# google-deepmind/dm_control

Measured on AMD Instinct MI355X. Metric: env-steps/s (whole node) at batch 4096; max rel qpos error vs CPU, higher is better.
Workload: dtype f32

## Files before the change

### dm_control_amd/csrc/step_core.h

```cpp
#pragma once
#include "../../include/dmc_model_layout.h"
#include "step_layout.h"
#include "step_defs.h"
#include "step_math.h"
#include "step_lanes.h"
#include "step_dense.h"
#include "step_geom.h"

namespace dmc {
#ifdef DMC_HOST_EMU
inline int& emu_split_solves() { static int n = 0; return n; }
inline long long* emu_ls_counts() { static long long n[6] = {0, 0, 0, 0, 0, 0}; return n; }
#endif

#if defined(DMC_PROFILE) && !defined(DMC_HOST_EMU)
#define DMC_PROF(id) do { if (lane == 0) { const int t_ = (int)__builtin_readcyclecounter(); SI(prof)[id] += t_ - SI(prof)[33]; SI(prof)[33] = t_; } } while (0)
#else
#define DMC_PROF(id) ((void)0)
#endif
#ifdef DMC_TRACE_SUB
#define DMC_TSUB(region, cond, row) do { if (DMC_TRACE_SUB == (region) && (cond)) sub_stamp(row); } while (0)
#else
#define DMC_TSUB(region, cond, row) ((void)0)
#endif
enum { PROF_LOAD = 0, PROF_KIN, PROF_COM, PROF_CRB, PROF_COLL, PROF_CONSTR, PROF_COMVEL, PROF_RNE, PROF_SENS, PROF_ACT,
       PROF_ACC, PROF_SOL_INIT, PROF_SOL_GRAD, PROF_SOL_LS, PROF_SOL_UPD, PROF_EULER, PROF_TRAIL, PROF_STORE,
       PROF_NOSLIP, PROF_HESS, PROF_FACTOR, PROF_SOLVE, PROF_LS_SETUP, PROF_X1, PROF_X2, PROF_X3, PROF_X4, PROF_X5, PROF_X6,
       PROF_X7, PROF_X8, PROF_N };

enum {
  OUT_SENSOR = 1 << 0, OUT_XPOS = 1 << 1, OUT_XQUAT = 1 << 2, OUT_XMAT = 1 << 3,
  OUT_XIPOS = 1 << 4, OUT_GEOM = 1 << 5, OUT_SITE = 1 << 6, OUT_SUBTREE_COM = 1 << 7,
  OUT_QACC = 1 << 8, OUT_ACTUATOR = 1 << 9, OUT_CONTACT = 1 << 10, OUT_QFRC = 1 << 11, OUT_CVEL = 1 << 12,
  OUT_CONTACT_IDS = 1 << 13,
  OUT_ALL = 0x7fffffff
};

enum LaunchMode { MODE_STEP = 0, MODE_FORWARD = 1, MODE_FORWARD_NOACT = 2, MODE_ROLLOUT = 3, MODE_STEP1 = 4, MODE_STEP2 = 5 };

template <typename T>
struct StepIO {
  int B;
  T *qpos, *qvel, *ctrl, *qacc_warmstart, *qfrc_applied;
  T *act;
  double* time;
  T *sensordata, *xpos, *xquat, *xmat, *xipos, *geom_xpos, *geom_xmat;
  T *site_xpos, *site_xmat, *subtree_com, *qacc, *actuator_force, *qfrc_actuator;
  T *qfrc_bias, *qfrc_constraint, *contact_dist, *contact_pos, *contact_frame;
  T *contact_force;
  T *cvel;
  int *ncon, *nefc, *solver_iter, *warning, *contact_geom1, *contact_geom2;
  const int* env_mode;
  int* work;
  int* cost; const int* order;
  int* prog = nullptr; int slices = 0; int nxcd = 1;
  unsigned long long* hand = nullptr; int hand_n = 0;
  const void* task_args = nullptr;
  int* trace; int trace_slot;
  T* probe = nullptr; int probe_geom = 0, probe_cap = 0;
  const T* ctrl_seq; T *qpos_seq, *qvel_seq, *sensor_seq;
  T* stash_r; int* stash_i; const int* epoch;
  T* kstash; int* kstash_i;
  long long* prof;
  T* debug;
  int* debug_i;
  int ndebug;
};

#ifndef DMC_STATIC_FEATURES
#define DMC_STATIC_FEATURES 1
#endif
template <typename T> struct LSPoint { T alpha, cost, d0, d1; };
template <typename T> DMC_DEV constexpr bool ls_relative() { return sizeof(T) == 4; }
template <typename T> DMC_DEV constexpr bool ls_anchored() { return ls_relative<T>(); }
#ifdef DMC_HOST_EMU
template <typename T> struct LSVec { T v[4]; DMC_DEV T operator[](int i) const { return v[i]; } };
#define DMC_LSVEC(T) LSVec<T>
#else
#define DMC_LSVEC(T) T __attribute__((ext_vector_type(4)))
#endif
template <typename T, int LPE>
DMC_FN DMC_LSVEC(T) ls_eval_lds(T a, const DMC_LDS T* jar_, const DMC_LDS T* jv_, const DMC_LDS T* D_,
                                T qg0, T qg1, T qg2, int nefc, int lane) {
  LSPoint<T> pt;
  LSPoint<T>* p = &pt;
  p->alpha = a;
  T q0 = 0, q1 = 0, q2 = 0;
  for (int i = lane; i < nefc; i += LPE) {
    const T jar = jar_[i], jv = jv_[i];
    if (ls_relative<T>()) {
      const bool act_a = jar + a*jv < 0, act_0 = jar < 0;
      if (act_a | act_0) {
        const T D = D_[i], dj0 = D*jar;
        if (act_a) { if (!ls_anchored<T>()) q1 += jv*dj0; q2 += (T)0.5*D*jv*jv; }
        if (act_a != act_0) { q0 += (act_a ? (T)0.5 : (T)-0.5)*jar*dj0; if (ls_anchored<T>()) q1 += act_a ? jv*dj0 : -(jv*dj0); }
      }
    } else if (jar + a*jv < 0) {
      const T D = D_[i], dj0 = D*jar;
      q0 += (T)0.5*jar*dj0; q1 += jv*dj0; q2 += (T)0.5*D*jv*jv;
    }
  }
  q0 = group_sum<LPE>(q0) + qg0; q1 = group_sum<LPE>(q1) + qg1; q2 = group_sum<LPE>(q2) + qg2;
  p->cost = a*a*q2 + a*q1 + q0;
  p->d0 = 2*a*q2 + q1;
  p->d1 = 2*q2;
  if (p->d1 <= 0) p->d1 = (T)DMC_MINVAL;
  DMC_LSVEC(T) rv = {pt.alpha, pt.cost, pt.d0, pt.d1};
  return rv;
}

struct DynLayoutSrc {
  static constexpr int kNV = 0;
  static constexpr int kJGlobal = -1;
  static constexpr int kNKin = 0;
  static constexpr int kTreeMax = 0;
  static constexpr int kTreeUni = 0;
  const StepLayout* p;
  DMC_DEV const StepLayout& get() const { return *p; }
};

#ifndef DMC_LS_SLOPE_ULPS
#define DMC_LS_SLOPE_ULPS 16
#endif
#ifndef DMC_PRIO_ITER
#define DMC_PRIO_ITER 2
#endif
template <typename T, int LPE, typename LS> struct StageFns;

template <typename T>
struct TaskLds { const T *qpos, *qvel, *ctrl, *act, *sensordata, *xpos, *xmat, *xipos, *subtree_com, *geom_xpos, *cvel; };

template <typename T, int LPE, typename LS = DynLayoutSrc>
struct StepCore {
  LS ls;
  const StepLayout& L;
  const StepOpts<T>& o;
  const int* mi;
  const T* mr;
  const int* gc;
  T* s;
  int* si;
  int lane;
  double time_;
  bool hsplit;


  DMC_DEV StepCore(LS ls_, const StepOpts<T>& o_, const int* mi_, const T* mr_, const int* gc_, T* s_, int* si_, int lane_)
      : ls(ls_), L(ls_.get()), o(o_), mi(mi_), mr(mr_),
#ifndef DMC_HOST_EMU
        gc(ls_.get().d.coldlds ? reinterpret_cast<const int*>(mr_ + ls_.get().n_mr_lds) : gc_),
#else
        gc(gc_),
#endif
        s(s_), si(si_), lane(lane_), time_(0), hsplit(false) {}

#define MI(n) (mi + L.mi_##n)
#define MR(n) (mr + L.mr_##n)
#define MRC(n) (mrc() + L.mr_##n)
#define MRS(n) ((L.d.sitegl ? (const T*)o.g_mr : (const T*)mr) + L.mr_##n)
#define GC(n) (gc + L.mc_##n)
#define S(n) (s + L.s_##n)
#define SG(n) (sg_##n())
#define SI(n) (si + L.si_##n)
#define FOR_LANES(i, n) for (int i = lane; i < (n); i += LPE)

// ... 2556 lines not shown
    chol_factor_inplace(S(qLH), nv, hsplit);
    DMC_PROF(PROF_FACTOR);
    chol_solve(S(sv_Mgrad), S(qLH), S(sv_grad), nv, hsplit);
    DMC_PROF(PROF_SOLVE);
  }
  DMC_DEV bool h_split(int nefc) {
    if (!L.d.treemax) return false;
    const RowMap rm = row_map();
    if (rm.s0 > 0 || rm.c0 > rm.tl0) return false;
    const int ncon = rm.c0 < nefc ? SI(imisc)[IM_NCON] : 0;
    int coupled = 0;
    for (int c = lane; c < ncon; c += LPE) {
      if (SI(con_efc)[c] < 0) continue;
      const unsigned lo = con_mask_lo(c), hi = con_mask_hi(c);
      if (!(lo | hi)) continue;
      const int first = lo ? __builtin_ctz(lo) : 32 + __builtin_ctz(hi);
      const int last = hi ? 63 - __builtin_clz(hi) : 31 - __builtin_clz(lo);
      if (last >= MI(dof_tree1)[first]) coupled = 1;
    }
    return group_max<LPE>(coupled) == 0;
  }
  typedef dmc::LSPoint<T> LSPoint;
  enum { LSK_NONE = 0, LSK_EQUALITY, LSK_FRICTION, LSK_ONESIDED, LSK_CONE };
#if !defined(DMC_NO_ROW_REDUCE)
  static constexpr int kRegsRed = LPE < 16 ? LPE : 16;
#else
  static constexpr int kRegsRed = LPE;
#endif
  struct LSRows { T jar, jv, D; bool on; bool gen; int kind; T f, rf, U0, V0, UU, UV, VV, mu, b0, b1, b2, Dm, NT0, T0; bool bottom0, middle0; };
  DMC_DEV void ls_load_gen(LSRows& g, int nefc) {
    g.gen = true; g.kind = LSK_NONE;
    g.f = g.rf = g.U0 = g.V0 = g.UU = g.UV = g.VV = g.mu = g.b0 = g.b1 = g.b2 = g.Dm = g.NT0 = g.T0 = 0; g.bottom0 = g.middle0 = false;
    const bool in = lane < nefc;
    const int i = in ? lane : 0;
    const int tid = SI(efc_tid)[i], ty = EFC_TYPE(tid), id = EFC_ID(tid);
    const bool ell = in && ty == EFC_ELLIPTIC;
    const int c = ell ? id : 0;
    const int r0 = SI(con_efc)[c], info = SI(con_info)[c];
    const bool head = ell && i == r0;
    T jr[6], jvv[6], Dr[6];
#pragma unroll
    for (int j = 0; j < 6; j++) {
#ifdef DMC_HOST_EMU
      const int rj = i + j < L.d.njmax ? i + j : i;
#else
      const int rj = i + j;
#endif
      jr[j] = S(efc_jar)[rj]; jvv[j] = S(efc_jv)[rj]; Dr[j] = S(efc_D)[rj];
    }
    const T floss = MR(dof_frictionloss)[(in && ty == EFC_FRICTION) ? id : 0];
    const T* fr = MR(prm_friction) + 3*(head ? prm_of_info(info) : 0);
    const T fr0 = fr[0], fr1 = fr[1], fr2 = fr[2];
    if (!in) return;
    g.jar = jr[0]; g.jv = jvv[0]; g.D = Dr[0];
    if (ty == EFC_EQUALITY) { g.kind = LSK_EQUALITY; return; }
    if (ty == EFC_FRICTION) { g.kind = LSK_FRICTION; g.f = floss; g.rf = g.f / g.D; return; }
    if (ty != EFC_ELLIPTIC) { g.kind = LSK_ONESIDED; return; }
    if (!head) return;
    g.kind = LSK_CONE;
    const int dim = info & 0xff;
    const T D0 = g.D;
    const T mu = fr0 * t_sqrt(D0 / Dr[1]);
    T UU = 0, UV = 0, VV = 0, b0 = 0, b1 = 0, b2 = 0;
#pragma unroll
    for (int j = 0; j < 6; j++) if (j < dim) {
      const T jar = jr[j], jv = jvv[j], D = Dr[j], dj0 = D*jar;
      b0 += (T)0.5*jar*dj0; b1 += jv*dj0; b2 += (T)0.5*D*jv*jv;
      if (j) {
        const T f = j < 3 ? fr0 : (j == 3 ? fr1 : fr2);
        const T u = jar*f, v = jv*f;
        UU += u*u; UV += u*v; VV += v*v;
      }
    }
    g.U0 = g.jar*mu; g.V0 = g.jv*mu; g.UU = UU; g.UV = UV; g.VV = VV; g.mu = mu; g.b0 = b0; g.b1 = b1; g.b2 = b2;
    g.Dm = D0 / t_max((T)DMC_MINVAL, mu*mu*(1 + mu*mu));
    if (UU <= 0) g.bottom0 = g.U0 < 0;
    else {
      const T T0 = t_sqrt(UU);
      if (g.U0 >= mu*T0) {}
      else if (mu*g.U0 + T0 <= 0) g.bottom0 = true;
      else { g.middle0 = true; g.NT0 = g.U0 - mu*T0; g.T0 = T0; }
    }
  }
  DMC_DEV void ls_eval_gen(LSPoint* p, const T* qg, const LSRows& g) {
    const T a = p->alpha;
    constexpr bool rel = ls_relative<T>();
    const bool anch = anchored();
    T q0 = 0, q1 = 0, q2 = 0, cc = 0, cd0 = 0, cd1 = 0;
    if (g.kind == LSK_EQUALITY) {
      const T dj0 = g.D*g.jar;
      if (!rel) q0 += (T)0.5*g.jar*dj0;
      if (!anch) q1 += g.jv*dj0;
      q2 += (T)0.5*g.D*g.jv*g.jv;
    } else if (g.kind == LSK_FRICTION) {
      const T jar = g.jar, jv = g.jv, D = g.D, f = g.f, rf = g.rf, x = jar + a*jv;
      const int za = x <= -rf ? -1 : (x >= rf ? 1 : 0), z0 = jar <= -rf ? -1 : (jar >= rf ? 1 : 0);
      if (za < 0) { q0 += f*((T)-0.5*rf - jar); if (!anch) q1 += -f*jv; }
      else if (za > 0) { q0 += f*((T)-0.5*rf + jar); if (!anch) q1 += f*jv; }
      else { const T dj0 = D*jar; q0 += (T)0.5*jar*dj0; if (!anch) q1 += jv*dj0; q2 += (T)0.5*D*jv*jv; }
      if (rel) {
        if (z0 < 0) q0 -= f*((T)-0.5*rf - jar);
        else if (z0 > 0) q0 -= f*((T)-0.5*rf + jar);
        else q0 -= (T)0.5*jar*D*jar;
      }
      if (anch && za != z0) q1 += (za < 0 ? -f*jv : (za > 0 ? f*jv : jv*(D*jar))) - (z0 < 0 ? -f*jv : (z0 > 0 ? f*jv : jv*(D*jar)));
    } else if (g.kind == LSK_ONESIDED) {
      const T jar = g.jar, jv = g.jv;
      if (rel) {
        const bool act_a = jar + a*jv < 0, act_0 = jar < 0;
        if (act_a | act_0) {
          const T D = g.D, dj0 = D*jar;
          if (act_a) { if (!anch) q1 += jv*dj0; q2 += (T)0.5*D*jv*jv; }
          if (act_a != act_0) { q0 += (act_a ? (T)0.5 : (T)-0.5)*jar*dj0; if (anch) q1 += act_a ? jv*dj0 : -(jv*dj0); }
        }
      } else if (jar + a*jv < 0) { const T D = g.D, dj0 = D*jar; q0 += (T)0.5*jar*dj0; q1 += jv*dj0; q2 += (T)0.5*D*jv*jv; }
    } else if (g.kind == LSK_CONE) {
      const T U0 = g.U0, V0 = g.V0, UU = g.UU, UV = g.UV, VV = g.VV, mu = g.mu, Dm = g.Dm;
      const T N = U0 + a*V0, Tsqr = UU + a*(2*UV + a*VV);
      bool bottom = false, middle = false;
      T NT = 0, NT1 = 0, Tn = 0;
      if (Tsqr <= 0) bottom = N < 0;
      else {
        Tn = t_sqrt(Tsqr);
        if (N >= mu*Tn) {}
        else if (mu*N + Tn <= 0) bottom = true;
        else {
          middle = true;
          const T N1 = V0, T1 = (UV + a*VV)/Tn, T2 = VV/Tn - (UV + a*VV)*T1/(Tn*Tn);
          NT1 = N1 - mu*T1;
          NT = N - mu*Tn;
          if (!rel) cc += (T)0.5*Dm*NT*NT;
          if (!anch) cd0 += Dm*NT*NT1;
          cd1 += Dm*(NT1*NT1 - NT*mu*T2);
        }
      }
      if (!rel) { if (bottom) { q0 += g.b0; q1 += g.b1; q2 += g.b2; } }
      else {
        if (bottom) { if (!anch || !g.bottom0) q1 += g.b1; q2 += g.b2; if (!g.bottom0) q0 += g.b0; }
        else if (g.bottom0) q0 -= g.b0;
        if (anch && g.bottom0 && !bottom) q1 -= g.b1;
        if (middle | g.middle0) {
          if (!anch) cc += (T)0.5*Dm*(NT - g.NT0)*(NT + g.NT0);
          else cone_middle_anchored(a, middle, g.middle0, Dm, NT, NT1, Tn, g.NT0, g.T0, V0, UV, VV, mu, &cc, &cd0);
        }
      }
    }
    q0 = group_sum<LPE>(q0) + (rel ? (T)0 : qg[0]); q1 = group_sum<LPE>(q1) + qg[1]; q2 = group_sum<LPE>(q2) + qg[2];
    cc = group_sum<LPE>(cc); cd0 = group_sum<LPE>(cd0); cd1 = group_sum<LPE>(cd1);
    p->cost = a*a*q2 + a*q1 + q0 + cc;
    p->d0 = 2*a*q2 + q1 + cd0;
    p->d1 = 2*q2 + cd1;
    if (p->d1 <= 0) p->d1 = (T)DMC_MINVAL;
  }
  template <int RED = LPE>
  DMC_DEV void ls_eval(LSPoint* p, const T* qg, int nefc, int* evals, const LSRows& rw) {
#ifdef DMC_HOST_EMU
    emu_ls_counts()[1]++;
#endif
    if (general_rows()) { if (rw.gen) ls_eval_gen(p, qg, rw); else ls_eval_ell(p, qg, nefc); (*evals)++; return; }
    if (rw.on) {
      const T a = p->alpha, jar = rw.jar, jv = rw.jv;
      T q0 = 0, q1 = 0, q2 = 0;
      if (ls_relative<T>()) {
        const bool act_a = jar + a*jv < 0, act_0 = jar < 0;
        if (act_a | act_0) {
          const T D = rw.D, dj0 = D*jar;
          if (act_a) { if (!ls_anchored<T>()) q1 += jv*dj0; q2 += (T)0.5*D*jv*jv; }
          if (act_a != act_0) { q0 += (act_a ? (T)0.5 : (T)-0.5)*jar*dj0; if (ls_anchored<T>()) q1 += act_a ? jv*dj0 : -(jv*dj0); }
        }
      } else if (jar + a*jv < 0) {
        const T D = rw.D, dj0 = D*jar;
        q0 += (T)0.5*jar*dj0; q1 += jv*dj0; q2 += (T)0.5*D*jv*jv;
      }
      q0 = group_sum<RED>(q0) + (ls_relative<T>() ? (T)0 : qg[0]); q1 = group_sum<RED>(q1) + qg[1]; q2 = group_sum<RED>(q2) + qg[2];
      p->cost = a*a*q2 + a*q1 + q0;
      p->d0 = 2*a*q2 + q1;
      p->d1 = 2*q2;
      if (p->d1 <= 0) p->d1 = (T)DMC_MINVAL;
      (*evals)++;
      return;
    }
    const DMC_LSVEC(T) rv = ls_eval_lds<T, LPE>(p->alpha, (const DMC_LDS T*)S(efc_jar), (const DMC_LDS T*)S(efc_jv),
                                                (const DMC_LDS T*)S(efc_D), ls_relative<T>() ? (T)0 : qg[0], qg[1], qg[2], nefc, lane);
    p->alpha = rv[0]; p->cost = rv[1]; p->d0 = rv[2]; p->d1 = rv[3];
    (*evals)++;
  }
  template <int RED = LPE>
  DMC_DEV int ls_update_bracket(LSPoint* p, const LSPoint* cand, LSPoint* pnext, const T* qg, int nefc, int* evals, const LSRows& rw) {
    int flag = 0;
    for (int i = 0; i < 3; i++) {
      if (p->d0 < 0 && cand[i].d0 < 0 && p->d0 < cand[i].d0) { *p = cand[i]; flag = 1; }
      else if (p->d0 > 0 && cand[i].d0 > 0 && p->d0 > cand[i].d0) { *p = cand[i]; flag = 2; }
    }
    if (flag) { pnext->alpha = p->alpha - p->d0/p->d1; ls_eval<RED>(pnext, qg, nefc, evals, rw); }
    return flag;
  }
  struct LSPre { T a1, a2, a3, a4, jar, jv, D; };
  template <bool REGS = false>
  DMC_DEV T primal_search(int nefc, T gauss, T scale, T* lscost, const LSPre& pre = LSPre()) {
    *lscost = 0;
    constexpr int RED = REGS ? kRegsRed : LPE;
#ifdef DMC_HOST_EMU
    emu_ls_counts()[0]++;
#endif
    const int nv = L.d.nv;
    if constexpr (!REGS) {
    mul_M(S(sv_Mv), S(sv_search));
    { const RowMap rm = row_map(); for (int i = lane; i < nefc; i += LPE) S(efc_jv)[i] = row_dot(i, S(sv_search), rm); }
    DMC_WSYNC();
    }
    LSRows rw;
    rw.jar = rw.jv = rw.D = 0; rw.on = false; rw.gen = false; rw.kind = LSK_NONE;
    if (general_rows() && nefc <= LPE && LPE > 1) ls_load_gen(rw, nefc);
    if (L.d.elliptic && !rw.gen) ls_prepare_ell(nefc);
    T a1 = 0, a2 = 0, a3 = 0, a4 = 0;
    const bool anch = anchored();
    if constexpr (REGS) { a1 = pre.a1; a2 = pre.a2; a3 = pre.a3; a4 = pre.a4; } else
    FOR_LANES(i, nv) {
      const T sr = S(sv_search)[i];
      if (anch) a1 += sr*S(sv_grad)[i];
      else { a1 += sr*S(sv_Ma)[i]; a2 += S(qfrc_smooth)[i]*sr; }
      a3 += sr*S(sv_Mv)[i]; a4 += sr*sr;
    }
    a1 = group_sum<RED>(a1); if (!anch) a2 = group_sum<RED>(a2); a3 = group_sum<RED>(a3); a4 = group_sum<RED>(a4);
    T qg[3] = {gauss, a1 - a2, (T)0.5*a3};
    const T snorm = t_sqrt(a4);
    if (snorm < (T)DMC_MINVAL) return 0;
    T gtol = o.tolerance * o.ls_tolerance * snorm / scale;
    const int lsmax = o.ls_iterations;
    int evals = 0;
#ifndef DMC_HOST_EMU
    if constexpr (REGS) { rw.on = true; rw.jar = pre.jar; rw.jv = pre.jv; rw.D = pre.D; } else
    if (!general_rows() && nefc <= LPE) {
      rw.on = true;
      if (lane < nefc) { rw.jar = S(efc_jar)[lane]; rw.jv = S(efc_jv)[lane]; rw.D = S(efc_D)[lane]; }
    }
#endif
    DMC_PROF(PROF_LS_SETUP);
    LSPoint p0, p1, p2, pmid, p1next, p2next;
    p0.alpha = 0; ls_eval<RED>(&p0, qg, nefc, &evals, rw);
#ifdef DMC_HOST_EMU
    { const char* u = getenv("DMC_LS_SLOPE_ULPS");
      if (sizeof(T) == 4) gtol = t_max(gtol, (T)((u ? atof(u) : (double)DMC_LS_SLOPE_ULPS) * 1.1920929e-7) * t_abs(p0.d0)); }
#else
    if (sizeof(T) == 4) gtol = t_max(gtol, (T)(DMC_LS_SLOPE_ULPS * 1.1920929e-7) * t_abs(p0.d0));
#endif
    p1.alpha = p0.alpha - p0.d0/p0.d1; ls_eval<RED>(&p1, qg, nefc, &evals, rw);
#ifdef DMC_HOST_EMU
    if (getenv("DMC_EMU_TRACE_LS")) fprintf(stderr, "    ls: p0 cost %.6e d0 %.6e d1 %.6e | p1 alpha %.9e cost %.6e d0 %.6e d1 %.6e | gtol %.3e qg1 %.6e\n",
                                           (double)p0.cost, (double)p0.d0, (double)p0.d1, (double)p1.alpha, (double)p1.cost, (double)p1.d0, (double)p1.d1, (double)gtol, (double)qg[1]);
#endif
    if (p0.cost < p1.cost) p1 = p0;
    if (t_abs(p1.d0) < gtol) { *lscost = p1.cost; return p1.alpha; }
    const int dir = p1.d0 < 0 ? 1 : -1;
    int p2update = 0;
    p2 = p1;
    while (p1.d0*dir <= -gtol && evals < lsmax) {
      p2 = p1; p2update = 1;
      p1.alpha -= p1.d0/p1.d1; ls_eval<RED>(&p1, qg, nefc, &evals, rw);
      if (t_abs(p1.d0) < gtol) { *lscost = p1.cost; return p1.alpha; }
    }
    if (evals >= lsmax) { *lscost = p1.cost; return p1.alpha; }
    if (!p2update) { *lscost = p1.cost; return p1.alpha; }
    p2next = p1;
    p1next.alpha = p1.alpha - p1.d0/p1.d1; ls_eval<RED>(&p1next, qg, nefc, &evals, rw);
    while (evals < lsmax) {
      pmid.alpha = (T)0.5*(p1.alpha + p2.alpha); ls_eval<RED>(&pmid, qg, nefc, &evals, rw);
      LSPoint cand[3] = {p1next, p2next, pmid};
      bool found = false; T best_cost = 0, best_alpha = 0;
      for (int i = 0; i < 3; i++) if (t_abs(cand[i].d0) < gtol && (!found || cand[i].cost < best_cost)) {
        found = true; best_cost = cand[i].cost; best_alpha = cand[i].alpha;
      }
      if (found) { *lscost = best_cost; return best_alpha; }
      const int b1 = ls_update_bracket<RED>(&p1, cand, &p1next, qg, nefc, &evals, rw);
      const int b2 = ls_update_bracket<RED>(&p2, cand, &p2next, qg, nefc, &evals, rw);
      if (!b1 && !b2) { if (pmid.cost < p0.cost) { *lscost = pmid.cost; return pmid.alpha; } return 0; }
    }
    if (p1.cost <= p2.cost && p1.cost < p0.cost) { *lscost = p1.cost; return p1.alpha; }
    if (p2.cost <= p1.cost && p2.cost < p0.cost) { *lscost = p2.cost; return p2.alpha; }
    return 0;
  }
  template <int N>
  DMC_DEV static int qcqp(T* res, const T* Ain, const T* bin, const T* dd, T r) {
    constexpr bool fast = sizeof(T) == 4;
    T A[N*N], b[N], Lc[N*N], inv[N], v[N], pv[N], la = 0;
#pragma unroll
    for (int i = 0; i < N; i++) { v[i] = 0; pv[i] = 0; inv[i] = 0; b[i] = bin[i]*dd[i]; }
#pragma unroll
    for (int i = 0; i < N; i++)
#pragma unroll
      for (int j = 0; j < N; j++) { A[i*N + j] = Ain[i*N + j]*dd[i]*dd[j]; Lc[i*N + j] = 0; }
    const T val_floor = fast ? t_max((T)1e-10, (T)(16*1.1920929e-7)*r*r) : (T)1e-10;
    bool fail = false;
    for (int iter = 0; iter < 20; iter++) {
#pragma unroll
      for (int i = 0; i < N; i++)
#pragma unroll
        for (int j = 0; j <= i; j++) {
          T t = A[i*N + j] + (i == j ? la : (T)0);
#pragma unroll
          for (int k = 0; k < j; k++) t -= Lc[i*N + k]*Lc[j*N + k];
          if (i == j) {
            if (t < (T)1e-10) fail = true;
            const T tc = t_max(t, (T)1e-30);
            if (fast) { inv[i] = t_rsqrt(tc); Lc[i*N + i] = tc*inv[i]; }
            else Lc[i*N + i] = t_sqrt(tc);
          } else Lc[i*N + j] = fast ? t*inv[j] : t/Lc[j*N + j];
        }
      if (fail) break;
#pragma unroll
      for (int i = 0; i < N; i++) {
        T t = -b[i];
#pragma unroll
        for (int k = 0; k < i; k++) t -= Lc[i*N + k]*v[k];
        v[i] = fast ? t*inv[i] : t/Lc[i*N + i];
      }
#pragma unroll
      for (int i = N - 1; i >= 0; i--) {
        T t = v[i];
#pragma unroll
        for (int k = i + 1; k < N; k++) t -= Lc[k*N + i]*v[k];
        v[i] = fast ? t*inv[i] : t/Lc[i*N + i];
      }
      T val = -r*r;
#pragma unroll
      for (int i = 0; i < N; i++) val += v[i]*v[i];
      if (val < val_floor) break;
#pragma unroll
      for (int i = 0; i < N; i++) {
        T t = v[i];
#pragma unroll
        for (int k = 0; k < i; k++) t -= Lc[i*N + k]*pv[k];
        pv[i] = fast ? t*inv[i] : t/Lc[i*N + i];
      }
      T deriv = 0;
#pragma unroll
      for (int i = 0; i < N; i++) deriv += pv[i]*pv[i];
      deriv *= -2;
      const T delta = -val/deriv;
      if (delta < (fast ? t_max((T)1e-10, (T)(4*1.1920929e-7)*la) : (T)1e-10)) break;
      la += delta;
#ifdef DMC_HOST_EMU
      emu_ls_counts()[5]++;
#endif
    }
#ifdef DMC_HOST_EMU
    emu_ls_counts()[4]++;
#endif
    if (fail) {
#pragma unroll
      for (int i = 0; i < N; i++) res[i] = 0;
      return 0;
    }
#pragma unroll
    for (int i = 0; i < N; i++) res[i] = v[i]*dd[i];
    return la != 0;
  }
  template <int N>
  DMC_DEV void noslip_block_solve(const T* Ac, const T* old, const T* bres, T* fnew, int t, int id) {
    if (N == 1) {
      const T fl = MR(dof_frictionloss)[id];
      fnew[0] = old[0] - bres[0]/Ac[0];
      if (fnew[0] < -fl) fnew[0] = -fl; else if (fnew[0] > fl) fnew[0] = fl;
    } else if (t == EFC_PYRAMIDAL) {
      const T bc0 = bres[0] - Ac[0]*old[0] - Ac[1]*old[N > 1 ? 1 : 0], bc1 = bres[N > 1 ? 1 : 0] - Ac[N > 1 ? N : 0]*old[0] - Ac[N > 1 ? N + 1 : 0]*old[N > 1 ? 1 : 0];
      const T mid = (T)0.5*(old[0] + old[N > 1 ? 1 : 0]);
      const T K1 = Ac[0] + Ac[N > 1 ? N + 1 : 0] - Ac[N > 1 ? 1 : 0] - Ac[N > 1 ? N : 0], K0 = mid*(Ac[0] - Ac[N > 1 ? N + 1 : 0]) + bc0 - bc1;
      T f0, f1;
      if (K1 < (T)DMC_MINVAL) f0 = f1 = mid;
      else {
        const T y = -K0/K1;
        if (y < -mid) { f0 = 0; f1 = 2*mid; }
        else if (y > mid) { f0 = 2*mid; f1 = 0; }
        else { f0 = mid + y; f1 = mid - y; }
      }
      fnew[0] = f0; fnew[N > 1 ? 1 : 0] = f1;
    } else {
      const T* fr3 = MR(prm_friction) + 3*con_prm(id);
      const T fri5[5] = {fr3[0], fr3[0], fr3[1], fr3[2], fr3[2]};
      T fri[N], bc[N];
#pragma unroll
      for (int p = 0; p < N; p++) fri[p] = fri5[p < 5 ? p : 4];
      const T fn = S(efc_force)[SI(con_efc)[id]];
#pragma unroll
      for (int p = 0; p < N; p++) {
        bc[p] = bres[p];
#pragma unroll
        for (int q = 0; q < N; q++) bc[p] -= Ac[p*N + q]*old[q];
      }
      if (fn >= (T)DMC_MINVAL) {
        const int active = qcqp<N>(fnew, Ac, bc, fri, fn);
        if (active) {
          T ss = 0;
#pragma unroll
          for (int p = 0; p < N; p++) ss += (fnew[p]/fri[p])*(fnew[p]/fri[p]);
          ss = t_sqrt(fn*fn / t_max((T)DMC_MINVAL, ss));
#pragma unroll
          for (int p = 0; p < N; p++) fnew[p] *= ss;
        }
      }
    }
  }
  template <int N>
  DMC_DEV T noslip_block(int a, int nf, int t, int id) {
    T Ac[N*N], old[N], bres[N], fnew[N];
#pragma unroll
    for (int p = 0; p < N; p++) {
      old[p] = S(efc_force)[SI(ns_row)[a + p]]; bres[p] = S(ns_res)[a + p]; fnew[p] = 0;
#pragma unroll
      for (int q = 0; q < N; q++) Ac[p*N + q] = ns_A()[(a + p)*L.d.nslip + a + q];
    }
    noslip_block_solve<N>(Ac, old, bres, fnew, t, id);
    T change = 0;
#pragma unroll
    for (int p = 0; p < N; p++) {
      T tq = 0;
#pragma unroll
      for (int q = 0; q < N; q++) tq += Ac[p*N + q]*(fnew[q] - old[q]);
      change += (T)0.5*(fnew[p] - old[p])*tq + (fnew[p] - old[p])*bres[p];
    }
    if (change > (T)1e-10) {
#pragma unroll
      for (int p = 0; p < N; p++) fnew[p] = old[p];
      change = 0;
    }
    DMC_WSYNC();
#pragma unroll
    for (int p = 0; p < N; p++) {
      const T delta = fnew[p] - old[p];
// ... 1421 lines not shown
```

### dm_control_amd/csrc/step_lanes.h

```cpp
#pragma once
#include "step_defs.h"

namespace dmc {
#ifndef DMC_HOST_EMU
template <int CTRL> DMC_DEV int dpp_i(int v) { return __builtin_amdgcn_update_dpp(0, v, CTRL, 0xF, 0xF, false); }
template <int CTRL> DMC_DEV float dpp_f(float v) { return __int_as_float(dpp_i<CTRL>(__float_as_int(v))); }
template <int CTRL> DMC_DEV double dpp_f(double v) {
  const long long b = __double_as_longlong(v);
  const int lo = dpp_i<CTRL>((int)(b & 0xffffffffll)), hi = dpp_i<CTRL>((int)(b >> 32));
  return __longlong_as_double(((long long)hi << 32) | (unsigned int)lo);
}
#endif
#ifndef DMC_HOST_EMU
struct Pair32 { unsigned a, b; };
DMC_DEV Pair32 swap16(unsigned x) { const auto r = __builtin_amdgcn_permlane16_swap(x, x, false, false); Pair32 p = {r[0], r[1]}; return p; }
DMC_DEV Pair32 swap32(unsigned x) { const auto r = __builtin_amdgcn_permlane32_swap(x, x, false, false); Pair32 p = {r[0], r[1]}; return p; }
template <int W> DMC_DEV Pair32 swapW(unsigned x) { return W == 16 ? swap16(x) : swap32(x); }
template <int W> DMC_DEV float xsum(float v) { const Pair32 p = swapW<W>(__float_as_uint(v)); return __uint_as_float(p.a) + __uint_as_float(p.b); }
template <int W> DMC_DEV int xsum(int v) { const Pair32 p = swapW<W>((unsigned)v); return (int)p.a + (int)p.b; }
template <int W> DMC_DEV double xsum(double v) {
  const unsigned long long u = __builtin_bit_cast(unsigned long long, v);
  const Pair32 lo = swapW<W>((unsigned)u), hi = swapW<W>((unsigned)(u >> 32));
  return __builtin_bit_cast(double, ((unsigned long long)hi.a << 32) | lo.a) + __builtin_bit_cast(double, ((unsigned long long)hi.b << 32) | lo.b);
}
template <int W> DMC_DEV int xmax(int v) { const Pair32 p = swapW<W>((unsigned)v); return (int)p.a > (int)p.b ? (int)p.a : (int)p.b; }
#endif
template <int LPE, typename V> DMC_DEV V group_sum(V v) {
#ifndef DMC_HOST_EMU
  if (LPE >= 2) v += dpp_f<0xB1>(v);
  if (LPE >= 4) v += dpp_f<0x4E>(v);
  if (LPE >= 8) v += dpp_f<0x141>(v);
  if (LPE >= 16) v += dpp_f<0x140>(v);
  if (LPE >= 32) v = xsum<16>(v);
  if (LPE >= 64) v = xsum<32>(v);
#endif
  return v;
}
#ifndef DMC_HOST_EMU
DMC_DEV float readlane_t(float v, int l) { return __builtin_bit_cast(float, __builtin_amdgcn_readlane(__builtin_bit_cast(int, v), l)); }
DMC_DEV int readlane_t(int v, int l) { return __builtin_amdgcn_readlane(v, l); }
DMC_DEV double readlane_t(double v, int l) {
  const unsigned long long u = __builtin_bit_cast(unsigned long long, v);
  const unsigned lo = (unsigned)__builtin_amdgcn_readlane((int)(unsigned)u, l);
  const unsigned hi = (unsigned)__builtin_amdgcn_readlane((int)(unsigned)(u >> 32), l);
  return __builtin_bit_cast(double, ((unsigned long long)hi << 32) | lo);
}
#endif
template <int LPE, typename V> DMC_DEV V wave_bcast(V v, int k) {
#ifndef DMC_HOST_EMU
  if (LPE == 64) return readlane_t(v, k);
  const int g = (int)(__lane_id()) / LPE;
  V r = readlane_t(v, k);
#pragma unroll
  for (int q = 1; q < 64 / LPE; q++) { const V w = readlane_t(v, q*LPE + k); r = g == q ? w : r; }
  return r;
#else
  (void)k; return v;
#endif
}
#ifndef DMC_HOST_EMU
template <int CTRL> DMC_DEV float dpp_all(float v) { return __int_as_float(__builtin_amdgcn_update_dpp(0, __float_as_int(v), CTRL, 0xF, 0xF, true)); }
template <int CTRL> DMC_DEV double dpp_all(double v) {
  const long long b = __double_as_longlong(v);
  const int lo = __builtin_amdgcn_update_dpp(0, (int)(b & 0xffffffffll), CTRL, 0xF, 0xF, true), hi = __builtin_amdgcn_update_dpp(0, (int)(b >> 32), CTRL, 0xF, 0xF, true);
  return __longlong_as_double(((long long)hi << 32) | (unsigned int)lo);
}
template <typename V> DMC_DEV V row_bcast16(V v, int k) {
  switch (k & 15) {
    case 0: return dpp_all<0x150>(v); case 1: return dpp_all<0x151>(v); case 2: return dpp_all<0x152>(v); case 3: return dpp_all<0x153>(v);
    case 4: return dpp_all<0x154>(v); case 5: return dpp_all<0x155>(v); case 6: return dpp_all<0x156>(v); case 7: return dpp_all<0x157>(v);
    case 8: return dpp_all<0x158>(v); case 9: return dpp_all<0x159>(v); case 10: return dpp_all<0x15A>(v); case 11: return dpp_all<0x15B>(v);
    case 12: return dpp_all<0x15C>(v); case 13: return dpp_all<0x15D>(v); case 14: return dpp_all<0x15E>(v); default: return dpp_all<0x15F>(v);
  }
}
#endif
template <int LPE, int N, typename V> DMC_DEV V bcast_rows(V v, int k) {
#if !defined(DMC_HOST_EMU) && !defined(DMC_NO_ROW_NEWBCAST)
  if constexpr (N <= 16 && LPE >= 16) return row_bcast16(v, k);
#endif
  return wave_bcast<LPE>(v, k);
}
template <int LPE> DMC_DEV int group_max(int v) {
#ifndef DMC_HOST_EMU
  int w;
  if (LPE >= 2) { w = dpp_i<0xB1>(v); v = w > v ? w : v; }
  if (LPE >= 4) { w = dpp_i<0x4E>(v); v = w > v ? w : v; }
  if (LPE >= 8) { w = dpp_i<0x141>(v); v = w > v ? w : v; }
  if (LPE >= 16) { w = dpp_i<0x140>(v); v = w > v ? w : v; }
  if (LPE >= 32) v = xmax<16>(v);
  if (LPE >= 64) v = xmax<32>(v);
#endif
  return v;
}
template <int LPE> DMC_DEV int group_scan(int v, int lane, int* total) {
#ifndef DMC_HOST_EMU
  int inc = v;
  (void)lane;
  if (LPE >= 2) inc += __builtin_amdgcn_update_dpp(0, inc, 0x111, 0xF, 0xF, true);
  if (LPE >= 4) inc += __builtin_amdgcn_update_dpp(0, inc, 0x112, 0xF, 0xF, true);
  if (LPE >= 8) inc += __builtin_amdgcn_update_dpp(0, inc, 0x114, 0xF, 0xF, true);
  if (LPE >= 16) inc += __builtin_amdgcn_update_dpp(0, inc, 0x118, 0xF, 0xF, true);
  if (LPE >= 32) inc += __builtin_amdgcn_update_dpp(0, inc, 0x142, 0xA, 0xF, false);
  if (LPE >= 64) inc += __builtin_amdgcn_update_dpp(0, inc, 0x143, 0xC, 0xF, false);
  *total = wave_bcast<LPE>(inc, LPE - 1);
  return inc - v;
#else
  (void)lane; *total = v; return 0;
#endif
}
}
```

Before: 80.34 million.

## Batch line-search evaluations into fused multi-point cross-lane reductions

The bracketing phase of the primal line search now evaluates the next p1, p2 and midpoint candidates together, and their partial sums go through one interleaved DPP reduction (group_sum_n) instead of separate serial reductions per point. Bracket updates are rewritten as branchless selects. The intent is to cut the latency of dependent cross-lane reduction chains and reduce divergent control flow in the line search. Evaluating the midpoint alongside the bracket updates reorders evals relative to the lsmax cap, and the explicit fma/contract-off arithmetic may shift results slightly versus the old path.

```diff
diff --git a/dm_control_amd/csrc/step_core.h b/dm_control_amd/csrc/step_core.h
--- a/dm_control_amd/csrc/step_core.h
+++ b/dm_control_amd/csrc/step_core.h
@@ -11,6 +11,7 @@
 #ifdef DMC_HOST_EMU
 inline int& emu_split_solves() { static int n = 0; return n; }
 inline long long* emu_ls_counts() { static long long n[6] = {0, 0, 0, 0, 0, 0}; return n; }
+inline long long* emu_ls_passes() { static long long n[3] = {0, 0, 0}; return n; }
 #endif
 
 #if defined(DMC_PROFILE) && !defined(DMC_HOST_EMU)
@@ -2873,12 +2874,68 @@
     p->d1 = 2*q2 + cd1;
     if (p->d1 <= 0) p->d1 = (T)DMC_MINVAL;
   }
+#if !defined(DMC_NO_LS_FUSED)
+  static constexpr bool kLsFused = true;
+#else
+  static constexpr bool kLsFused = false;
+#endif
+#if !defined(DMC_HOST_EMU)
+  DMC_DEV static T ls_fma(T a, T b, T c) {
+#pragma clang fp contract(off)
+    if constexpr (sizeof(T) == 4) return __builtin_fmaf(a, b, c);
+    else return a*b + c;
+  }
+  DMC_DEV static void ls_terms_regs(T a, const LSRows& rw, T* q0, T* q1, T* q2) {
+#pragma clang fp contract(off)
+    const T jar = rw.jar, jv = rw.jv, D = rw.D, dj0 = D*jar, zero = 0;
+    const T x = ls_fma(a, jv, jar);
+    const bool act_a = x < 0, act_0 = jar < 0, sw = act_a != act_0;
+    const T h2 = zero + (T)0.5*D*jv*jv, h1 = jv*dj0;
+    if (ls_relative<T>()) {
+      const T h0 = zero + (act_a ? (T)0.5 : (T)-0.5)*jar*dj0;
+      *q0 = sw ? h0 : zero;
+      if (ls_anchored<T>()) { const T s1 = zero + (act_a ? h1 : -h1); *q1 = sw ? s1 : zero; }
+      else { const T s1 = zero + h1; *q1 = act_a ? s1 : zero; }
+      *q2 = act_a ? h2 : zero;
+    } else {
+      const T h0 = zero + (T)0.5*jar*dj0, s1 = zero + h1;
+      *q0 = act_a ? h0 : zero; *q1 = act_a ? s1 : zero; *q2 = act_a ? h2 : zero;
+    }
+  }
+  DMC_DEV static void ls_point_regs(LSPoint* p, T a, T s0, T s1, T s2, const T* qg) {
+#pragma clang fp contract(off)
+    const T q0 = s0 + (ls_relative<T>() ? (T)0 : qg[0]), q1 = s1 + qg[1], q2 = s2 + qg[2];
+    p->cost = ls_fma(a, q1, a*a*q2) + q0;
+    p->d0 = 2*a*q2 + q1;
+    p->d1 = 2*q2;
+    if (p->d1 <= 0) p->d1 = (T)DMC_MINVAL;
+  }
+  template <int K, int RED>
+  DMC_DEV static void ls_points_regs(const T (&al)[K], LSPoint (&r)[K], const T* qg, const LSRows& rw) {
+    T s[3*K];
+#pragma unroll
+    for (int k = 0; k < K; k++) ls_terms_regs(al[k], rw, &s[k], &s[K + k], &s[2*K + k]);
+    group_sum_n<RED, 3*K>(s);
+#pragma unroll
+    for (int k = 0; k < K; k++) { r[k].alpha = al[k]; ls_point_regs(&r[k], al[k], s[k], s[K + k], s[2*K + k], qg); }
+  }
+#endif
   template <int RED = LPE>
   DMC_DEV void ls_eval(LSPoint* p, const T* qg, int nefc, int* evals, const LSRows& rw) {
 #ifdef DMC_HOST_EMU
-    emu_ls_counts()[1]++;
+    emu_ls_counts()[1]++; emu_ls_passes()[0]++;
 #endif
     if (general_rows()) { if (rw.gen) ls_eval_gen(p, qg, rw); else ls_eval_ell(p, qg, nefc); (*evals)++; return; }
+#if !defined(DMC_HOST_EMU)
+    if (kLsFused && rw.on) {
+      const T al[1] = {p->alpha};
+      LSPoint r[1];
+      ls_points_regs<1, RED>(al, r, qg, rw);
+      *p = r[0];
+      (*evals)++;
+      return;
+    }
+#endif
     if (rw.on) {
       const T a = p->alpha, jar = rw.jar, jv = rw.jv;
       T q0 = 0, q1 = 0, q2 = 0;
@@ -2915,6 +2972,53 @@
     }
     if (flag) { pnext->alpha = p->alpha - p->d0/p->d1; ls_eval<RED>(pnext, qg, nefc, evals, rw); }
     return flag;
+  }
+  DMC_DEV static int ls_pick_bracket(LSPoint* p, const LSPoint* cand) {
+    int flag = 0;
+    LSPoint q = *p;
+#pragma unroll
+    for (int i = 0; i < 3; i++) {
+      const LSPoint c = cand[i];
+      const bool lo = (q.d0 < 0) & (c.d0 < 0) & (q.d0 < c.d0), hi = (q.d0 > 0) & (c.d0 > 0) & (q.d0 > c.d0), take = lo | hi;
+      flag = lo ? 1 : (hi ? 2 : flag);
+      q.alpha = take ? c.alpha : q.alpha; q.cost = take ? c.cost : q.cost; q.d0 = take ? c.d0 : q.d0; q.d1 = take ? c.d1 : q.d1;
+    }
+    *p = q;
+    return flag;
+  }
+  template <int RED = LPE>
+  DMC_DEV void ls_eval_multi(LSPoint* pa, LSPoint* pb, LSPoint* pc, bool ea, bool eb, bool ec, const T* qg, int nefc, int* evals, const LSRows& rw) {
+#if !defined(DMC_HOST_EMU)
+    if (!general_rows() && rw.on) {
+      const int n = (ea ? 1 : 0) + (eb ? 1 : 0) + (ec ? 1 : 0);
+      *evals += n;
+      if (n == 3) {
+        T al[3] = {pa->alpha, pb->alpha, pc->alpha};
+        LSPoint r[3];
+        ls_points_regs<3, RED>(al, r, qg, rw);
+        *pa = r[0]; *pb = r[1]; *pc = r[2];
+      } else if (n == 2) {
+        T al[2] = {ea ? pa->alpha : pb->alpha, ec ? pc->alpha : pb->alpha};
+        LSPoint r[2];
+        ls_points_regs<2, RED>(al, r, qg, rw);
+        if (ea) *pa = r[0]; else *pb = r[0];
+        if (ec) *pc = r[1]; else *pb = r[1];
+      } else if (n == 1) {
+        T al[1] = {ea ? pa->alpha : (eb ? pb->alpha : pc->alpha)};
+        LSPoint r[1];
+        ls_points_regs<1, RED>(al, r, qg, rw);
+        if (ea) *pa = r[0]; else if (eb) *pb = r[0]; else *pc = r[0];
+      }
+      return;
+    }
+#endif
+    if (ea) ls_eval<RED>(pa, qg, nefc, evals, rw);
+    if (eb) ls_eval<RED>(pb, qg, nefc, evals, rw);
+    if (ec) ls_eval<RED>(pc, qg, nefc, evals, rw);
+#ifdef DMC_HOST_EMU
+    const int n = (ea ? 1 : 0) + (eb ? 1 : 0) + (ec ? 1 : 0);
+    if (n > 1) { emu_ls_passes()[0] -= n - 1; emu_ls_passes()[2]++; }
+#endif
   }
   struct LSPre { T a1, a2, a3, a4, jar, jv, D; };
   template <bool REGS = false>
@@ -2984,6 +3088,32 @@
     if (evals >= lsmax) { *lscost = p1.cost; return p1.alpha; }
     if (!p2update) { *lscost = p1.cost; return p1.alpha; }
     p2next = p1;
+#ifdef DMC_HOST_EMU
+    emu_ls_passes()[1]++;
+#endif
+    if constexpr (kLsFused) {
+      bool e1 = true, e2 = false;
+      p1next.alpha = p1.alpha - p1.d0/p1.d1;
+      for (;;) {
+        const bool mid = evals + (e1 ? 1 : 0) + (e2 ? 1 : 0) < lsmax;
+        pmid.alpha = (T)0.5*(p1.alpha + p2.alpha);
+        ls_eval_multi<RED>(&p1next, &p2next, &pmid, e1, e2, mid, qg, nefc, &evals, rw);
+        if (!mid) break;
+        LSPoint cand[3] = {p1next, p2next, pmid};
+        bool found = false; T best_cost = 0, best_alpha = 0;
+#pragma unroll
+        for (int i = 0; i < 3; i++) {
+          const bool ok = (t_abs(cand[i].d0) < gtol) & (!found | (cand[i].cost < best_cost));
+          best_cost = ok ? cand[i].cost : best_cost; best_alpha = ok ? cand[i].alpha : best_alpha; found |= ok;
+        }
+        if (found) { *lscost = best_cost; return best_alpha; }
+        const int b1 = ls_pick_bracket(&p1, cand), b2 = ls_pick_bracket(&p2, cand);
+        if (!b1 && !b2) { if (pmid.cost < p0.cost) { *lscost = pmid.cost; return pmid.alpha; } return 0; }
+        e1 = b1 != 0; e2 = b2 != 0;
+        if (e1) p1next.alpha = p1.alpha - p1.d0/p1.d1;
+        if (e2) p2next.alpha = p2.alpha - p2.d0/p2.d1;
+      }
+    } else {
     p1next.alpha = p1.alpha - p1.d0/p1.d1; ls_eval<RED>(&p1next, qg, nefc, &evals, rw);
     while (evals < lsmax) {
       pmid.alpha = (T)0.5*(p1.alpha + p2.alpha); ls_eval<RED>(&pmid, qg, nefc, &evals, rw);
@@ -2996,6 +3126,7 @@
       const int b1 = ls_update_bracket<RED>(&p1, cand, &p1next, qg, nefc, &evals, rw);
       const int b2 = ls_update_bracket<RED>(&p2, cand, &p2next, qg, nefc, &evals, rw);
       if (!b1 && !b2) { if (pmid.cost < p0.cost) { *lscost = pmid.cost; return pmid.alpha; } return 0; }
+    }
     }
     if (p1.cost <= p2.cost && p1.cost < p0.cost) { *lscost = p1.cost; return p1.alpha; }
     if (p2.cost <= p1.cost && p2.cost < p0.cost) { *lscost = p2.cost; return p2.alpha; }
diff --git a/dm_control_amd/csrc/step_lanes.h b/dm_control_amd/csrc/step_lanes.h
--- a/dm_control_amd/csrc/step_lanes.h
+++ b/dm_control_amd/csrc/step_lanes.h
@@ -35,6 +35,18 @@
   if (LPE >= 64) v = xsum<32>(v);
 #endif
   return v;
+}
+template <int LPE, int N, typename V> DMC_DEV void group_sum_n(V (&v)[N]) {
+#ifndef DMC_HOST_EMU
+#define DMC_EACH(expr) _Pragma("unroll") for (int k = 0; k < N; k++) { expr; asm("" : "+v"(v[k])); }
+  if (LPE >= 2) DMC_EACH(v[k] += dpp_f<0xB1>(v[k]))
+  if (LPE >= 4) DMC_EACH(v[k] += dpp_f<0x4E>(v[k]))
+  if (LPE >= 8) DMC_EACH(v[k] += dpp_f<0x141>(v[k]))
+  if (LPE >= 16) DMC_EACH(v[k] += dpp_f<0x140>(v[k]))
+  if (LPE >= 32) DMC_EACH(v[k] = xsum<16>(v[k]))
+  if (LPE >= 64) DMC_EACH(v[k] = xsum<32>(v[k]))
+#undef DMC_EACH
+#endif
 }
 #ifndef DMC_HOST_EMU
 DMC_DEV float readlane_t(float v, int l) { return __builtin_bit_cast(float, __builtin_amdgcn_readlane(__builtin_bit_cast(int, v), l)); }
```

Result: faster. 81.74 million (median of 6 runs) (+1.7%).
